# mpieva/network-aware-bwa

Hardware: AMD Instinct MI355X
Metric: aligned reads/s to GRCh38 (100 bp SE), FM-index search (bwa_cal_sa_reg_gap), bit-exact vs CPU (higher is better)
Workload: dtype u32

## Files before the change

include/nabwa.h:

```cpp
#ifndef NABWA_H
#define NABWA_H
#include <stdint.h>
#include <stddef.h>

#ifdef __cplusplus
extern "C" {
#endif

#define NABWA_OK        0
#define NABWA_ENODEV   -1
#define NABWA_EINVAL   -2
#define NABWA_EIO      -3
#define NABWA_ENOMEM   -4
#define NABWA_ECAP     -5
#define NABWA_EHITS    -6

typedef struct {
	int s_mm, s_gapo, s_gape;
	int mode;
	int indel_end_skip, max_del_occ, max_entries;
	float fnr;
	int max_diff, max_gapo, max_gape;
	int max_seed_diff, seed_len;
	int n_threads;
// ... 7 lines not shown
#define NABWA_MODE_NONSTOP  0x10

typedef struct { uint32_t info; uint32_t k, l; int32_t score; } nabwa_aln1_t;

typedef struct nabwa_index nabwa_index_t;

const char *nabwa_last_error(void);
int nabwa_device_count(void);

void nabwa_gap_init_opt(nabwa_gap_opt_t *opt);
int nabwa_cal_maxdiff(int len, double err, double thres);

int nabwa_index_load(const char *prefix, int device, int with_sa, int with_pac, nabwa_index_t **out);

int nabwa_index_from_arrays(int device, int is_device, const uint32_t *bwt0, uint64_t n_words0,
							const uint32_t *bwt1, uint64_t n_words1, const uint32_t *sa0, uint64_t n_sa_words0,
							const uint32_t *sa1, uint64_t n_sa_words1, nabwa_index_t **out);
void nabwa_index_destroy(nabwa_index_t *ix);
uint32_t nabwa_index_seq_len(const nabwa_index_t *ix, int which);
uint64_t nabwa_index_device_bytes(const nabwa_index_t *ix);

int nabwa_cal_sa_reg_gap(nabwa_index_t *ix, const nabwa_gap_opt_t *opt, int n, const int64_t *off,
						 const uint8_t *seq, const uint8_t *rseq, int per_read,
						 int32_t *n_aln, nabwa_aln1_t *aln_out, int64_t aln_cap, int64_t *n_rows,
						 int32_t *max_entries);

typedef struct nabwa_batch nabwa_batch_t;
int nabwa_batch_create(nabwa_index_t *ix, const nabwa_gap_opt_t *opt, int n, const int64_t *off,
					   const uint8_t *seq, const uint8_t *rseq, int per_read, nabwa_batch_t **out);
int nabwa_batch_run(nabwa_batch_t *b);
int nabwa_batch_sync(nabwa_batch_t *b, int *n_second_pass);
float nabwa_batch_last_kernel_ms(nabwa_batch_t *b);
float nabwa_batch_last_width_ms(nabwa_batch_t *b);
float nabwa_batch_last_deep_ms(nabwa_batch_t *b);
int nabwa_batch_count_touches(nabwa_batch_t *b, uint64_t *n_bucket, uint64_t *n_bucket_width);
int nabwa_batch_fetch(nabwa_batch_t *b, int32_t *n_aln, nabwa_aln1_t *aln_out, int64_t aln_cap, int64_t *n_rows,
					  int32_t *max_entries);
int nabwa_batch_width_records(nabwa_batch_t *b, int first, int n, uint32_t *w_out, uint8_t *bid_out, uint8_t *seed_bid_out);
int nabwa_batch_checksum(nabwa_batch_t *b, uint64_t *sum, int64_t *n_rows);
typedef struct {
	int32_t n, min_len, max_len;
	int32_t deep_only;
	int32_t ns1, ns_wide;
	int32_t w_sync;
	int32_t trip_budget, trip_budget_hard;
	int32_t n_sync;
	int32_t hard_budget;
	int32_t cls[3];
	int32_t coop_lanes;
	int32_t lds_rd;
} nabwa_batch_config_t;
int nabwa_batch_config(nabwa_batch_t *b, nabwa_batch_config_t *out);
int nabwa_batch_sure0_stats(nabwa_batch_t *b, uint64_t out[4]);
void nabwa_batch_destroy(nabwa_batch_t *b);

typedef struct { double avg, std, ap_prior; uint32_t low, high, high_bayesian; } nabwa_isize_t;
int nabwa_isize_infer(const uint16_t *hist, double ap_prior, int64_t L, nabwa_isize_t *out);
int nabwa_isize_bin(int kind, int mapq0, int mapq1, uint32_t pos0, int len0, uint32_t pos1, int len1);
typedef struct { uint32_t pos; int32_t strand, mapQ, seQ, len, full_len, n_mm, n_gapo, n_gape, score, extra_flag; } nabwa_pe_end_t;
int nabwa_pairing(nabwa_pe_end_t p[2], int n_hits, uint64_t *hits, const nabwa_aln1_t *rows0, const nabwa_aln1_t *rows1,
				  int max_isize, int s_mm, const nabwa_isize_t *ii);

typedef struct {
	char *name;
	uint8_t *seq, *rseq, *qual;
	uint32_t bits0, bits1;
	int32_t score, clip_len;
	int32_t n_aln; int32_t pad0;
	nabwa_aln1_t *aln;
	int32_t n_multi; int32_t pad1;
	void *multi;
	uint32_t sa, pos;
	uint64_t c1c2seq;
	int32_t n_cigar; int32_t pad2;
	uint16_t *cigar;
	int32_t tid;
	char bc[64];
	uint32_t lenbits;
	char *md;
	int32_t max_entries; int32_t pad3;
} nabwa_bwa_seq_t;

int nabwa_bwa_cal_sa_reg_gap(nabwa_index_t *ix, int n_seqs, nabwa_bwa_seq_t *seqs, const nabwa_gap_opt_t *opt);

int nabwa_encode_read(int full_len, const uint8_t *codes, const uint8_t *qual, int reverse, int trim_qual, int is_comp,
					  uint8_t *seq_out, uint8_t *rseq_out);

int nabwa_sa_lookup(nabwa_index_t *ix, int n, const uint8_t *which, const uint32_t *k, uint32_t *sa_out);

int nabwa_global_align(int device, int n, const int64_t *ref_off, const uint8_t *ref, const int64_t *qry_off,
					   const uint8_t *qry, int gap_open, int gap_ext, int gap_end, const int *matrix25, int band,
					   int32_t *score, int32_t *n_cigar, uint32_t *cigar32, int max_cigar);

void nabwa_dp_scratch_release(int device);

void nabwa_dp_form_counts(uint64_t *out, int n);

int nabwa_extend_align(int device, int n, const int64_t *ref_off, const uint8_t *ref, const int64_t *qry_off,
					   const uint8_t *qry, int gap_open, int gap_ext, const int *matrix25, int band, const int32_t *G0,
					   int32_t *score, int32_t *n_cigar, uint32_t *cigar32, int max_cigar);

int nabwa_local_align(int device, int n, const int64_t *ref_off, const uint8_t *ref, const int64_t *qry_off,
					  const uint8_t *qry, int gap_open, int gap_ext, const int *matrix25, int band, int thres,
					  int32_t *score, int32_t *coords, int32_t *subo, int32_t *n_cigar, uint32_t *cigar32, int max_cigar);

#define NABWA_MAX_CIGAR 64
// ... 176 lines not shown
```

network-aware-bwa_amd/__init__.py:

```python
import ctypes as C
import os
import subprocess

import numpy as np

_HERE = os.path.dirname(os.path.abspath(__file__))
LIB_PATH = os.environ.get("NABWA_LIB", os.path.join(_HERE, "libnabwa.so"))

OK, ENODEV, EINVAL, EIO, ENOMEM, ECAP, EHITS = 0, -1, -2, -3, -4, -5, -6

ALN_DT = np.dtype([("info", "<u4"), ("k", "<u4"), ("l", "<u4"), ("score", "<i4")])


class GapOpt(C.Structure):
    _fields_ = [("s_mm", C.c_int), ("s_gapo", C.c_int), ("s_gape", C.c_int), ("mode", C.c_int),
                ("indel_end_skip", C.c_int), ("max_del_occ", C.c_int), ("max_entries", C.c_int),
                ("fnr", C.c_float), ("max_diff", C.c_int), ("max_gapo", C.c_int), ("max_gape", C.c_int),
                ("max_seed_diff", C.c_int), ("seed_len", C.c_int), ("n_threads", C.c_int),
                ("max_top2", C.c_int), ("trim_qual", C.c_int)]


MAX_CIGAR, MAX_MD, MAX_MULTI = 64, 512, 16


# ... 190 lines not shown
        super().__init__("libnabwa error %d: %s" % (code, msg))
        self.code = code


def build(verbose=False):
    r = subprocess.run(["make", "-C", os.path.join(_HERE, "csrc"), "all"], capture_output=not verbose, text=True)
    if r.returncode != 0:
        raise RuntimeError("building libnabwa.so failed:\n%s\n%s" % (r.stdout, r.stderr))


_lib = None
_P = C.c_void_p


def lib():
    global _lib
    if _lib is not None:
        return _lib
    if not os.path.exists(LIB_PATH):
        raise RuntimeError("libnabwa.so is missing (%s): run __graft_entry__.build() / make -C %s"
                           % (LIB_PATH, os.path.join(_HERE, "csrc")))
    L = C.CDLL(LIB_PATH)
    L.nabwa_last_error.restype = C.c_char_p
    L.nabwa_device_count.restype = C.c_int
    L.nabwa_gap_init_opt.argtypes = [_P]
    L.nabwa_cal_maxdiff.restype = C.c_int
    L.nabwa_cal_maxdiff.argtypes = [C.c_int, C.c_double, C.c_double]
    L.nabwa_index_load.argtypes = [C.c_char_p, C.c_int, C.c_int, C.c_int, _P]
    L.nabwa_index_from_arrays.argtypes = [C.c_int, C.c_int, _P, C.c_uint64, _P, C.c_uint64, _P, C.c_uint64, _P,
                                          C.c_uint64, _P]
    L.nabwa_index_destroy.argtypes = [_P]
    L.nabwa_index_destroy.restype = None
    L.nabwa_index_seq_len.restype = C.c_uint32
    L.nabwa_index_seq_len.argtypes = [_P, C.c_int]
    L.nabwa_index_device_bytes.restype = C.c_uint64
    L.nabwa_index_device_bytes.argtypes = [_P]
    L.nabwa_cal_sa_reg_gap.argtypes = [_P, _P, C.c_int, _P, _P, _P, C.c_int, _P, _P, C.c_int64, _P, _P]
    L.nabwa_batch_create.argtypes = [_P, _P, C.c_int, _P, _P, _P, C.c_int, _P]
    L.nabwa_batch_run.argtypes = [_P]
    L.nabwa_batch_sync.argtypes = [_P, _P]
    L.nabwa_batch_last_kernel_ms.restype = C.c_float
    L.nabwa_batch_last_kernel_ms.argtypes = [_P]
    L.nabwa_batch_last_width_ms.restype = C.c_float
    L.nabwa_batch_last_width_ms.argtypes = [_P]
    L.nabwa_batch_last_deep_ms.restype = C.c_float
    L.nabwa_batch_last_deep_ms.argtypes = [_P]
    L.nabwa_batch_fetch.argtypes = [_P, _P, _P, C.c_int64, _P, _P]
    L.nabwa_batch_checksum.argtypes = [_P, _P, _P]
    L.nabwa_batch_count_touches.argtypes = [_P, _P, _P]
    L.nabwa_batch_config.argtypes = [_P, _P]
    if hasattr(L, "nabwa_batch_sure0_stats"):
        L.nabwa_batch_sure0_stats.restype = C.c_int
        L.nabwa_batch_sure0_stats.argtypes = [_P, _P]
    L.nabwa_dp_form_counts.argtypes = [_P, C.c_int]
    L.nabwa_dp_form_counts.restype = None
    L.nabwa_batch_destroy.argtypes = [_P]
    L.nabwa_batch_destroy.restype = None
    L.nabwa_sa_lookup.argtypes = [_P, C.c_int, _P, _P, _P]
    L.nabwa_occ4.argtypes = [_P, C.c_int, C.c_int, _P, _P]
    L.nabwa_global_align.argtypes = [C.c_int, C.c_int, _P, _P, _P, _P, C.c_int, C.c_int, C.c_int, _P, C.c_int, _P, _P, _P,
                                     C.c_int]
    L.nabwa_extend_align.argtypes = [C.c_int, C.c_int, _P, _P, _P, _P, C.c_int, C.c_int, _P, C.c_int, _P, _P, _P, _P, C.c_int]
    L.nabwa_local_align.argtypes = [C.c_int, C.c_int, _P, _P, _P, _P, C.c_int, C.c_int, _P, C.c_int, C.c_int, _P, _P, _P, _P, _P,
                                    C.c_int]
    L.nabwa_index_attach_reference.argtypes = [_P, C.c_char_p]
    L.nabwa_bwa_cal_sa_reg_gap.argtypes = [_P, C.c_int, _P, _P]
    L.nabwa_isize_infer.argtypes = [_P, C.c_double, C.c_int64, _P]
    L.nabwa_isize_bin.argtypes = [C.c_int, C.c_int, C.c_int, C.c_uint32, C.c_int, C.c_uint32, C.c_int]
    L.nabwa_pairing.argtypes = [_P, C.c_int, _P, _P, _P, C.c_int, C.c_int, _P]
    L.nabwa_encode_read.restype = C.c_int
    L.nabwa_encode_read.argtypes = [C.c_int, _P, _P, C.c_int, C.c_int, C.c_int, _P, _P]
    L.nabwa_se_finish.argtypes = [_P, _P, C.c_int, _P, _P, _P, _P, _P, _P, C.c_int, _P, _P]
    L.nabwa_index_export.argtypes = [_P, C.c_int, C.c_int, C.c_uint64, C.c_uint64, _P]
    L.nabwa_pe_opt_default.argtypes = [_P]
    L.nabwa_pe_opt_default.restype = None
    L.nabwa_pe_posn.argtypes = [_P, _P, C.c_int, _P, _P, _P, _P, _P, _P]
    L.nabwa_pe_finish.argtypes = [_P, _P, _P, _P, C.c_int, _P, _P, _P, _P, _P, _P, _P, _P]
    L.nabwa_index_fa2pac.restype = C.c_int64
    L.nabwa_index_fa2pac.argtypes = [C.c_char_p, C.c_char_p]
    L.nabwa_index_fa2cspac.restype = C.c_int64
    L.nabwa_index_fa2cspac.argtypes = [C.c_char_p, C.c_char_p]
    L.nabwa_index_build.argtypes = [C.c_char_p, C.c_int, C.c_int, C.c_int]
    L.nabwa_index_build_estimate.argtypes = [C.c_uint64, _P]
    L.nabwa_cs2nt.argtypes = [C.c_int, C.c_int, _P, _P, _P, _P]
    L.nabwa_index_attach_nt_reference.argtypes = [_P, C.c_char_p]
    L.nabwa_se_finish_cs.argtypes = [_P, _P, C.c_int, _P, _P, _P, _P, _P, _P, _P, C.c_int, _P, _P, _P, _P, _P, _P]
    L.nabwa_pe_finish_sampe_cs.argtypes = [_P, _P, _P, _P, C.c_int, _P, _P, _P, _P, _P, _P, _P, _P, _P, _P, _P, _P, _P]
    L.nabwa_pairing_typed.argtypes = [_P, C.c_int, _P, _P, _P, C.c_int, C.c_int, _P, C.c_int]
    L.nabwa_bgzf_bound.restype = C.c_int64
    L.nabwa_bgzf_bound.argtypes = [C.c_int64]
    L.nabwa_bgzf_compress.argtypes = [C.c_int, _P, C.c_int64, _P, C.c_int64, _P, _P]
    L.nabwa_bgzf_create.argtypes = [C.c_int, _P]
    L.nabwa_bgzf_handle_compress.argtypes = [_P, _P, C.c_int64, _P, C.c_int64, _P, _P]
    L.nabwa_bgzf_destroy.argtypes = [_P]
    L.nabwa_bgzf_destroy.restype = None
    _lib = L
    return L


def _chk(rc):
    if rc != OK:
        raise NabwaError(rc, lib().nabwa_last_error().decode())


def _ptr(a):
    return a.ctypes.data_as(_P) if a is not None else None
# ... 324 lines not shown
        s = C.c_uint64()
        r = C.c_int64()
        _chk(lib().nabwa_batch_checksum(self._h, C.byref(s), C.byref(r)))
        return s.value, r.value

    def count_touches(self):
        v, w = C.c_uint64(), C.c_uint64()
        _chk(lib().nabwa_batch_count_touches(self._h, C.byref(v), C.byref(w)))
        return v.value, w.value

    def fetch(self):
        n_aln = np.zeros(max(self.n, 1), np.int32)
        maxe = np.zeros(max(self.n, 1), np.int32)
        rows = C.c_int64()
        rc = lib().nabwa_batch_fetch(self._h, _ptr(n_aln), None, 0, C.byref(rows), _ptr(maxe))
        if rc not in (OK, ECAP):
            _chk(rc)
        buf = np.zeros(max(rows.value, 1), ALN_DT)
        if rows.value:
            _chk(lib().nabwa_batch_fetch(self._h, _ptr(n_aln), _ptr(buf), rows.value, C.byref(rows), _ptr(maxe)))
        n_aln = n_aln[:self.n]
        bounds = np.concatenate([[0], np.cumsum(n_aln)])
        return [buf[bounds[i]:bounds[i + 1]] for i in range(self.n)], maxe[:self.n]

    def fetch_flat(self, keep=None):
        if keep is not None and "n_aln" in keep and len(keep["n_aln"]) >= max(self.n, 1):
            n_aln, maxe, buf = keep["n_aln"], keep["maxe"], keep["rows"]
        else:
            n_aln = np.zeros(max(self.n, 1), np.int32)
            maxe = np.zeros(max(self.n, 1), np.int32)
            buf = None
        rows = C.c_int64()
        rc = lib().nabwa_batch_fetch(self._h, _ptr(n_aln), _ptr(buf) if buf is not None else None, len(buf) if buf is not None else 0, C.byref(rows), _ptr(maxe))
        if rc not in (OK, ECAP):
            _chk(rc)
        if rc == ECAP or buf is None:
            buf = np.zeros(max(rows.value + rows.value // 8, 1), ALN_DT)
            if rows.value:
                _chk(lib().nabwa_batch_fetch(self._h, _ptr(n_aln), _ptr(buf), len(buf), C.byref(rows), _ptr(maxe)))
        if keep is not None:
            keep["n_aln"], keep["maxe"], keep["rows"] = n_aln, maxe, buf
        return n_aln[:self.n], buf[:rows.value], maxe[:self.n]

    def config(self):
        c = BatchConfig()
        _chk(lib().nabwa_batch_config(self._h, C.byref(c)))
        return {f: (list(getattr(c, f)) if f == "cls" else getattr(c, f)) for f, _ in BatchConfig._fields_}

    def sure0_stats(self):
        out = (C.c_uint64 * 4)()
        _chk(lib().nabwa_batch_sure0_stats(self._h, out))
        return [int(x) for x in out]

    def close(self):
        if self._h:
            lib().nabwa_batch_destroy(self._h)
            self._h = None
```

network-aware-bwa_amd/csrc/fm_search.hip:

```cpp
#include "nabwa_dev.hpp"
#include "fm_search.hpp"
#include "launchers.hpp"

#define ST_IDLE   0
#define ST_WIDTH  1
#define ST_POP    2
#define ST_EXACT  3
#define ST_EXPAND 4
#define ST_EXIT   5

#define STATE_M 0
#define STATE_I 1
#define STATE_D 2
#define STATE_GROUP 3
#define GRP_EXT 0x100u
#define TXM 0xfffffffeu
#define KEYM 0xffffffffu
#define LVO(t_) ((size_t)((((uint64_t)1 << (2 * (t_))) - 4ull) / 3ull))
#ifndef NABWA_W_WAVES
#define NABWA_W_WAVES 5
#endif
#ifndef NABWA_WORK_CHUNK
#define NABWA_WORK_CHUNK 64u
#endif
// ... 196 lines not shown
				if (kk > ll || cc > 3) { kk = 0; ll = BX(seq_len); ++bid; rekey(wi + 1); }
				else if (was_one) { tmode = true; tp = sav - 1u; twtag = 0xffffffffu; }
			}
			out_pos(wi, false);
			if (wi + 1 == n) out_pos(wi + 1, true);
			++wi;
			if (wi == n) {
				if (phase == 0 && P.rd_cls) P.rd_cls[2 * (size_t)rid + x] = (uint8_t)(bid - 1 > 4 ? 4 : bid - 1);
				if (phase == 0 && len > P.seed_len) {
					phase = 1; wi = 0; n = P.seed_len; sbase = len - P.seed_len; tmode = false;
					if (KT) { wkey = P.rd_key[6 * (size_t)rid + 4 + x]; tok = wkey != 0xffffffffu; }
					tbase = 0;
					kk = 0; ll = BX(seq_len); bid = 0; pw = 0;
				} else { if (x == 0u) P.rd_nN[rid] = (uint8_t)(nN > 255 ? 255 : nN); run = false; }
			}
		}
	}
	if (COUNT) {
		for (int o = 32; o > 0; o >>= 1) touches += __shfl_down(touches, o);
		if (lane == 0 && P.touch_counter) atomicAdd(P.touch_counter + 1, touches);
	}
#undef WREC
#undef BX
}
#define LS_IDLE  0
#define LS_POP   1
#define LS_HAVE  2
#define LS_EXACT 3
#define LS_EXIT  4

template <bool COUNT>
__global__ __launch_bounds__(NABWA_SEARCH_BLOCK, NABWA_MIN_WAVES) void fm_search_kernel(const SearchParams P_)
{
	SearchParams P = P_;
	own(P.n); own(P.s_mm); own(P.s_gapo); own(P.s_gape); own(P.mode); own(P.indel_end_skip); own(P.max_del_occ); own(P.max_entries);
	own(P.max_gape); own(P.max_seed_diff); own(P.seed_len); own(P.max_top2);
	const uint32_t NIL = 0xffffu;
	const uint32_t lane = threadIdx.x & 63u;
	const size_t slot = (size_t)blockIdx.x * NABWA_SEARCH_BLOCK + threadIdx.x;
	uint8_t *const sc = P.scratch + slot * P.lane_stride;
	uint4 *const ent = (uint4*)sc;
	const bool gape_mode = P.mode & 0x01, nonstop = P.mode & 0x10, loggap = P.mode & 0x04;

	int st = LS_IDLE;
	unsigned int w_next = 0, w_end = 0; bool w_sync = false;
	uint32_t item = 0; int len = 0; uint32_t mdmg = 0;
	uint32_t sq_off = 0;
	const int KT = (int)P.bwt[0].kmer_T;
	uint32_t budget = P.trip_budget;
	if (!COUNT && P.n_sync && P.trip_budget_hard && 2u * (uint32_t)__builtin_amdgcn_readfirstlane((int)*P.n_sync) > (uint32_t)P.n) budget = P.trip_budget_hard;
#define RID item
#define REC (P.wdata + (size_t)RID * P.wstride)
#define MD_READ ((int)(mdmg & 0xffu))
#define MG_READ ((int)(mdmg >> 8 & 0x7fu))
	uint32_t k = 0, l = 0;
	int max_diff = 0, best_score = 0, best_cnt = 0, n_aln = 0, max_ent = 0, n_entries = 0;
	uint32_t bump = 0; uint64_t mask_lo = 0; bool seeded = false; int status = 0;
	int e_i = 0, e_a = 0, e_mm = 0, e_go = 0, e_ge = 0, e_state = 0, e_ldp = 0, e_score = 0, m = 0;
	uint4 pe = make_uint4(0, 0, 0, 0); int p_score = -1;
#define p_valid (p_score >= 0)
	int sq_tag = -1;
	int bw_base = -1, bw_a = -1;
	int sw_base = -1, sw_a = -1;
	unsigned long long touches = 0; uint32_t rd_touch = 0, rd_trips = 0;
	uint32_t rk_kf = 0, rk_row2 = 0, rk_row1 = 0, rk_tx = 0, rk_pop = 0, rk_tail = 0, rk_jump = 0, rk_gap = 0;
	unsigned long long st_trips = 0, st_expand = 0, st_exact = 0, st_ent = 0, st_spec = 0, st_query = 0, st_two = 0, st_exit = 0, st_jump = 0, st_txe = 0, st_txt = 0;
	bool ovf = false;
#define s0f mdmg
#define S0_ON  0x80000000u
#define S0_LAND 0x40000000u
#define S0_WAS 0x8000u

	auto head_get = [&](int score) -> uint32_t {
		return (uint32_t)s_head[score * NABWA_SEARCH_BLOCK + threadIdx.x];
	};
	auto head_set = [&](int score, uint32_t v) {
		s_head[score * NABWA_SEARCH_BLOCK + threadIdx.x] = (uint16_t)v;
	};
	auto mask_has = [&](int score) -> bool { return mask_lo >> score & 1ull; };
	auto mask_set = [&](int score) { mask_lo |= 1ull << score; };
	auto mask_clr = [&](int score) { mask_lo &= ~(1ull << score); };
	auto mask_any = [&]() -> bool { return mask_lo != 0ull; };
	auto mask_first = [&]() -> int {
		return mask_lo ? __ffsll((unsigned long long)mask_lo) - 1 : 0x7fffffff;
	};
	auto never_popped = [&](int score) -> bool { return !nonstop && score > best_score + P.s_mm; };
	auto mk_entry = [&](uint32_t nk, uint32_t nl, int ni, int nldp, int nmm, int ngo, int nge, int nstate, int na) -> uint4 {
		const uint32_t z = (uint32_t)ni | (uint32_t)nldp << 16;
		return make_uint4(nk, nl, z, (uint32_t)nmm << 16 | (uint32_t)ngo << 20 | (uint32_t)nge << 24 | (uint32_t)nstate << 29 | (uint32_t)na << 31);
	};
	auto push_mem = [&](int score, uint4 e) {
		if (ovf || never_popped(score)) return;
		if ((uint32_t)score >= P.NS) { ovf = true; return; }
		if (bump >= P.cap) { ovf = true; return; }
		const uint32_t s = bump++;
		const uint32_t prev = mask_has(score) ? head_get(score) : NIL;
		e.w |= prev;
		ent[s] = e;
		head_set(score, s);
		mask_set(score);
	};

	uint4 *const s_pf = (uint4*)(s_head + (size_t)P.NS * NABWA_SEARCH_BLOCK);
	uint2 *const s_key = (uint2*)(s_pf + NABWA_SEARCH_BLOCK);
	uint2 *const s_tw = s_key + NABWA_SEARCH_BLOCK;
	uint32_t *const s_bw = (uint32_t*)(s_tw + NABWA_SEARCH_BLOCK), *const s_sw = s_bw + 4 * NABWA_SEARCH_BLOCK, *const s_sq = s_sw + 4 * NABWA_SEARCH_BLOCK;
	uint32_t *const s_fb = s_sq + 4 * NABWA_SEARCH_BLOCK;
	auto win_byte = [&](const uint32_t *W, uint32_t idx) -> uint32_t {
		return (uint32_t)((const uint8_t*)W)[(threadIdx.x << 4) + idx];
	};
	auto win_load = [&](const void *src, uint32_t *W) {
		__builtin_amdgcn_global_load_lds((const void __attribute__((address_space(1)))*)src,
										 (void __attribute__((address_space(3)))*)(W + ((threadIdx.x & ~63u) << 2)), 16, 0, 0);
	};
#define BW_BYTE(i_) win_byte(s_bw, (uint32_t)(i_))
#define SW_BYTE(i_) win_byte(s_sw, (uint32_t)(i_))
#define SQ_BYTE(i_) win_byte(s_sq, (uint32_t)(i_))
	const bool kf_ok = KT > 0 && (int)P.bwt[0].kmer_LW == KT && (int)P.bwt[1].kmer_LW == KT && (P.text_mode & 4);
	const bool text_ok = (P.text_mode & 2) && P.bwt[0].sa_full && P.bwt[1].sa_full && P.bwt[0].seq_len < 0xfffffff0u;
	uint32_t pf_slot = NIL;
	bool finish = false;
	auto unpack = [&](const uint4 &r) {
		k = r.x; l = r.y; e_i = (int)(r.z & 0xffffu); e_ldp = (int)(r.z >> 16);
		e_mm = (int)(r.w >> 16 & 15u); e_go = (int)(r.w >> 20 & 15u); e_ge = (int)(r.w >> 24 & 31u);
		e_state = (int)(r.w >> 29 & 3u); e_a = (int)(r.w >> 31);
	};
	auto take_entry = [&](const uint4 &r_ent) {
		unpack(r_ent);
		const uint32_t nx = r_ent.w & 0xffffu;
		head_set(e_score, nx);
		if (nx == NIL) mask_clr(e_score);
		--n_entries;
		if (!nonstop && e_score > best_score + P.s_mm) finish = true;
	};

	for (;;) {
		finish = false;
		unsigned long long need = __ballot(st == LS_IDLE);
		const bool any_busy = __ballot(st != LS_IDLE && st != LS_EXIT) != 0ull;
		if ((P.sync_refill || w_sync) && any_busy) need = 0ull;
		if (need) {
			if (w_next == w_end) {
				unsigned int b0 = 0;
				if (lane == 0) b0 = atomicAdd(P.work_counter, (unsigned int)NABWA_WORK_CHUNK);
				w_next = __builtin_amdgcn_readfirstlane(b0); w_end = w_next + NABWA_WORK_CHUNK;
				w_sync = P.n_sync && (w_next >= *P.n_sync || w_next < P.n_sync[-8]);
			}
			const unsigned int rank = (unsigned int)__popcll(need & ((1ull << lane) - 1ull)), avail = w_end - w_next;
			const unsigned int base = w_next;
			w_next += min((unsigned int)__popcll(need), avail);
			if (st == LS_IDLE && rank < avail) {
				const unsigned int idx = base + rank;
				if (idx < (unsigned int)P.n) {
					const uint32_t rid = P.ids ? (uint32_t)P.ids[idx] : idx;
					item = rid;
					const int64_t o = P.poff[rid];
					len = P.rd_len[rid];
					sq_off = (uint32_t)o;
					mdmg = (uint32_t)P.rd_maxdiff[rid] | (uint32_t)P.rd_maxgapo[rid] << 8;
					if (KT) {
						s_key[threadIdx.x] = *(const uint2*)(P.rd_key + 6 * (size_t)rid);
						uint32_t fb = 0xffffu;
						if (len > KT) { const uint8_t *const bb = REC + P.woff_bid + (len - KT - 1); fb = (uint32_t)(bb[0] & 127u) | (uint32_t)(bb[P.WLB] & 127u) << 8; }
						s_fb[threadIdx.x] = fb;
					}
					n_aln = 0; max_ent = 0; status = NABWA_ST_OK; rd_touch = 0; rd_trips = 0; ovf = false;
					rk_kf = rk_row2 = rk_row1 = rk_tx = rk_pop = rk_tail = rk_jump = rk_gap = 0;
					sq_tag = -1; bw_a = -1; sw_a = -1; p_score = -1; pf_slot = NIL;
					if (text_ok) s_tw[threadIdx.x] = make_uint2(0u, 0x7fffffffu);
					if (!COUNT && P.sure0 && P.rd_cls && !nonstop && P.s_gapo > P.s_mm && MD_READ >= 1 && len > 0 && 2 + 4 * len <= P.max_entries) {
						const uint32_t cw = *(const uint16_t*)(P.rd_cls + 2 * (size_t)rid);
						if ((cw & 0xffu) == 0u || (cw >> 8) == 0u) {
							s0f |= P.sure0 > 1 ? S0_ON | S0_LAND | S0_WAS : S0_ON | S0_WAS;
						}
					}
					if (len > 0 && (int)P.rd_nN[rid] <= MD_READ) {
						seeded = len > P.seed_len;
						max_diff = MD_READ;
						best_score = (s0f & S0_ON) ? 0 : (MD_READ + 1) * P.s_mm + (MG_READ + 1) * P.s_gapo + (P.max_gape + 1) * P.s_gape;
						best_cnt = 0;
						bump = 0; mask_lo = 0ull;
						push_mem(0, mk_entry(0u, kf_ok ? KEYM : P.bwt[0].seq_len, len, 0, 0, 0, 0, STATE_M, 0));
						pe = mk_entry(0u, kf_ok ? KEYM : P.bwt[0].seq_len, len, 0, 0, 0, 0, STATE_M, 1); p_score = 0;
						n_entries = 2;
						st = LS_POP;
					} else { P.n_aln[item] = 0; P.max_ent[item] = 0; P.status[item] = NABWA_ST_OK; }
				} else st = LS_EXIT;
			}
		}
		if (__ballot(st != LS_EXIT) == 0ull) break;

		bool want_ent = false; uint32_t ent_slot = 0;
		bool have = st == LS_HAVE;
		if (st == LS_POP) {
			if (n_entries == 0) finish = true;
			else {
				if (max_ent < n_entries) max_ent = n_entries;
				if (n_entries > P.max_entries) finish = true;
				else if (!COUNT && P.trip_budget && rd_trips > budget) { status = NABWA_ST_OVERFLOW; finish = true; }
			}
			if (!finish) {
				const int best_mem = mask_first();
				if (p_valid && p_score <= best_mem) {
					unpack(pe);
					e_score = p_score; p_score = -1;
					--n_entries;
					if (!nonstop && e_score > best_score + P.s_mm) finish = true;
					else have = true;
				} else if (best_mem == 0x7fffffff) {
					finish = true;
				} else {
					if (p_valid) { push_mem(p_score, pe); p_score = -1; }
					if (ovf) { status = NABWA_ST_OVERFLOW; finish = true; }
					else {
						ent_slot = head_get(best_mem); e_score = best_mem;
						if (ent_slot == pf_slot) {
							const uint4 r = s_pf[threadIdx.x];
							take_entry(r);
							pf_slot = NIL;
							if (!finish) have = true;
						} else want_ent = true;
					}
				}
			}
		}
		int kind = 0;
		bool need_win = false, spec = false, forced = false; int win_hi = 0;
		int grp_c = 0, mlev = -1, mpost = 0; uint32_t midx = 0; bool kx = false;
		if (have && !finish && e_state == STATE_GROUP) {
			const uint32_t mk = (uint32_t)e_ldp & 0x1fu, ext = (uint32_t)e_ldp & GRP_EXT, more = (uint32_t)e_ldp >> 9;
			const int j = 31 - __clz((int)mk);
			const uint32_t rest = mk & ~(1u << j);
			if (rest) push_mem(e_score, mk_entry(k, l, e_i, (int)(rest | ext | more << 9), e_mm, e_go, e_ge, STATE_GROUP, e_a));
			else if (more) push_mem(e_score, mk_entry(k + 1u, l, e_i + 1, (int)(3u | (more - 1u) << 9), e_mm, e_go, e_ge, STATE_GROUP, e_a));
			if (ovf) { status = NABWA_ST_OVERFLOW; finish = true; }
			if (ext) ++e_ge; else ++e_go;
			if (l == KEYM) {
				const int dp = len - e_i - 1;
				kind = 6; st = LS_POP; have = false;
				if (j == 0) { mpost = 1; mlev = dp; midx = k; } else { mpost = 2; mlev = dp + 1; midx = k * 4u + (uint32_t)(j - 1); }
			}
			else if (j == 0) { e_state = STATE_I; e_ldp = e_i; }
			else if (l == TXM) { k -= 1u; e_i += 1; e_state = STATE_D; e_ldp = e_i; }
			else { kind = 5; grp_c = j - 1; st = LS_POP; have = false; }
		}
		if (have && !finish) {
			st = LS_POP;
			m = max_diff - (e_mm + e_go); if (gape_mode) m -= e_ge;
			if (m >= 0) {
				const bool kf = l == KEYM;
				const int d = len - e_i;
				if (e_i == 0) { if (kf) { kind = 6; mlev = d; midx = k; } else kind = 3; }
				else {
					const bool tail = m == 0 && (e_state == STATE_M || gape_mode || e_ge == P.max_gape);
					const bool landed = e_state == STATE_M && e_ldp > e_i;
					win_hi = landed ? e_ldp - 1 : e_i - 1;
					const int win_lo = landed ? win_hi : ((tail || e_i < 2) ? e_i - 1 : e_i - 2);
					bool go = true;
					if (bw_a == e_a && win_lo >= bw_base && win_hi < bw_base + 16) {
						if (m < (int)(BW_BYTE(win_hi - bw_base) & 127u)) go = false;
					} else { need_win = true; spec = true; }
					if (go) {
						const bool rdkey_ok = KT && (e_a ? s_key[threadIdx.x].y : s_key[threadIdx.x].x) != 0xffffffffu;
						const bool row_known = l != TXM && !kf && (e_go | e_ge) == 0 && e_state == STATE_M && (e_mm == 0 || (e_mm == 1 && e_ldp == e_i));
						if (tail) {
							kind = 2;
							if (l == TXM) kind = 7;
							else if (kf) { if (rdkey_ok) kind = 4; else { kind = 6; mlev = d; midx = k; } }
							else if (rdkey_ok && row_known && d <= KT) kind = 4;
						}
						else {
							forced = rdkey_ok && d < KT && (kf || row_known) && (int)(s_fb[threadIdx.x] >> (e_a << 3) & 0xffu) == m;
							if (forced) kind = 4;
							else if (kf && d >= KT) { kind = 6; mlev = d; midx = k; }
							else {
								kind = 1; --e_i; kx = kf;
								if ((s0f & S0_ON) && n_entries + 4 * len > P.max_entries) s0f &= ~S0_ON;
							}
						}
					}
				}
			}
		} else if (st == LS_EXACT) kind = l == TXM ? 7 : 2;
		auto rows_arrived = [&](uint32_t nk, uint32_t nl) {
			k = nk; l = nl;
			if (mpost == 1) { e_state = STATE_I; e_ldp = e_i; }
			else if (mpost == 2) { e_i += 1; e_state = STATE_D; e_ldp = e_i; }
			st = LS_HAVE;
		};
		if (kind == 6 && mlev == 0) { rows_arrived(0u, e_a ? P.bwt[0].seq_len : P.bwt[1].seq_len); kind = 0; }

		const int qb = 1 - e_a;
		const bool tx = l == TXM && (kind == 1 || kind == 3 || kind == 7);
		const int spos = (kind == 2 || kind == 7) ? e_i - 1 : e_i;
		const int stag = (e_a << 20) | (spos >> 4);
		const bool need_seq = (kind == 1 || kind == 2 || kind == 7) && stag != sq_tag;
		bool query = (kind == 1 && !tx && !kx) || kind == 2 || kind == 5;
		uint2 tw = make_uint2(0u, 0u); bool need_tw = false;
		if (tx && kind != 3 && k > 0u) {
			const uint32_t tag = ((k - 1u) >> 4) | (uint32_t)qb << 31;
			tw = s_tw[threadIdx.x];
			need_tw = tw.y != tag;
			tw.y = tag;
		}
		const bool to_text = kind == 1 && !tx && !kx && text_ok && k == l;
		if (kind == 2 && !need_seq && SQ_BYTE((uint32_t)spos & 15u) > 3u) query = false;
		const int ii = e_i - (len - P.seed_len);
		const bool use_seed = kind == 1 && e_i > 0 && seeded && ii > 0;
		const bool need_seed = use_seed && !(sw_a == e_a && ii - 1 >= sw_base && ii < sw_base + 16);

		uint4 r_ent = make_uint4(0, 0, 0, 0);
		if (need_win) {
			int base = (win_hi | 7) - 15; if (base < 0) base = 0;
			win_load(REC + P.woff_bid + e_a * P.WLB + base, s_bw); bw_base = base; bw_a = e_a;
		}
		if (need_seq) {
			win_load((e_a ? P.rseq : P.seq) + sq_off + (spos & ~15), s_sq); sq_tag = stag;
		}
		if (need_seed) {
			int base = (ii | 7) - 15; if (base < 0) base = 0;
			win_load(REC + P.woff_sbid + e_a * P.SLB + base, s_sw); sw_base = base; sw_a = e_a;
		}
		uint32_t r_x = 0u;
		if (need_tw) r_x = (qb ? P.bwt[1].text : P.bwt[0].text)[(k - 1u) >> 4];
		else if (tx && kind == 3) r_x = (qb ? P.bwt[1].isa : P.bwt[0].isa)[k];
		else if (to_text) r_x = (qb ? P.bwt[1].sa_full : P.bwt[0].sa_full)[k];
		uint2 r_km = make_uint2(1u, 0u);
		uint4 a0, a1, a2, a3, b0, b1, b2, b3;
// ... 276 lines not shown
								ek = gk; el = gl; ei = len - KT; s0f += 1u << 23;
							}
						}
						if (dead) ++n_entries;
						else emit(sc0 + (is_mm ? P.s_mm : 0), ek, el, ei, is_mm ? e_i : 0, e_mm + (is_mm ? 1 : 0), e_go, e_ge, STATE_M, 1);
						if (!is_mm) match_child = true;
					}
				}
			} else if (c < 4) {
				const uint32_t nk = L2Q(c) + CK(c) + 1u, nl = L2Q(c) + CL(c);
				if (nk <= nl) { emit(sc0, nk, nl, e_i, 0, e_mm, e_go, e_ge, STATE_M, 1); match_child = true; }
			}
			if (to_text && match_child) { pe.x = r_x - 1u; pe.y = TXM; }
			if (ovf) { status = NABWA_ST_OVERFLOW; finish = true; }
		}
#undef L2Q
#undef CK
#undef CL

		if (finish) {
			const bool net = (s0f & S0_ON) && status == NABWA_ST_OK && n_aln == 0;
			if (net) status = NABWA_ST_OVERFLOW;
			if (P.s0_stats && (s0f & S0_WAS)) atomicAdd(P.s0_stats, 1ull);
			if (P.s0_stats && (s0f >> 16 & 0x3fffu)) {
				atomicAdd(P.s0_stats + 1, (unsigned long long)(s0f >> 16 & 0x7fu)); atomicAdd(P.s0_stats + 2, (unsigned long long)(s0f >> 23 & 0x7fu));
			}
			if (P.s0_stats && net) atomicAdd(P.s0_stats + 3, 1ull);
			P.n_aln[item] = n_aln; P.max_ent[item] = (!COUNT && status == NABWA_ST_OVERFLOW) ? (int)rd_trips : max_ent; P.status[item] = (uint8_t)status;
			if (COUNT && status == NABWA_ST_OK) touches += rd_touch;
			if (COUNT && P.touch_counter && rd_trips > 8000u) {
				atomicAdd(P.touch_counter + 16, 1ull); atomicAdd(P.touch_counter + 17, (unsigned long long)rd_trips); atomicAdd(P.touch_counter + 18, (unsigned long long)rk_kf);
				atomicAdd(P.touch_counter + 19, (unsigned long long)rk_row2); atomicAdd(P.touch_counter + 20, (unsigned long long)rk_row1); atomicAdd(P.touch_counter + 21, (unsigned long long)rk_tx);
				atomicAdd(P.touch_counter + 22, (unsigned long long)rk_pop); atomicAdd(P.touch_counter + 23, (unsigned long long)rk_tail); atomicAdd(P.touch_counter + 24, (unsigned long long)rk_jump); atomicAdd(P.touch_counter + 25, (unsigned long long)rk_gap);
			}
			if (COUNT && P.touch_counter) { atomicMax(P.touch_counter + 13, (unsigned long long)rd_trips); if (rd_trips > 2000u) atomicAdd(P.touch_counter + 14, 1ull); if (rd_trips > 500u) atomicAdd(P.touch_counter + 15, 1ull); }
			st = LS_IDLE;
		}
	}
	if (COUNT) {
		for (int o = 32; o > 0; o >>= 1) touches += __shfl_down(touches, o);
		if (lane == 0 && P.touch_counter) {
			atomicAdd(P.touch_counter, touches);
			atomicAdd(P.touch_counter + 2, st_trips); atomicAdd(P.touch_counter + 3, st_expand); atomicAdd(P.touch_counter + 4, st_exact);
			atomicAdd(P.touch_counter + 5, st_ent); atomicAdd(P.touch_counter + 6, st_spec); atomicAdd(P.touch_counter + 7, st_query);
			atomicAdd(P.touch_counter + 8, st_two); atomicAdd(P.touch_counter + 9, st_exit); atomicAdd(P.touch_counter + 10, st_jump); atomicAdd(P.touch_counter + 11, st_txe); atomicAdd(P.touch_counter + 12, st_txt);
		}
	}
}

#undef p_valid
#undef S0_ON
#undef S0_LAND
#undef S0_WAS
#undef s0f
#undef BW_BYTE
#undef SW_BYTE
#undef SQ_BYTE
#undef RID
#undef REC
#undef MD_READ
#undef MG_READ
extern "C" void nabwa_launch_fm_width(const SearchParams *P, int n_blocks, hipStream_t s)
{
	if (P->touch_counter) hipLaunchKernelGGL((fm_width_kernel<true>), dim3(n_blocks), dim3(NABWA_SEARCH_BLOCK), 0, s, *P);
	else hipLaunchKernelGGL((fm_width_kernel<false>), dim3(n_blocks), dim3(NABWA_SEARCH_BLOCK), 0, s, *P);
}

extern "C" int nabwa_width_occupancy(void)
{
	int nb = 0;
	return hipOccupancyMaxActiveBlocksPerMultiprocessor(&nb, fm_width_kernel<false>, NABWA_SEARCH_BLOCK, 0) == hipSuccess ? nb : 0;
}

extern "C" void nabwa_launch_fm_search(const SearchParams *P, int n_blocks, hipStream_t s)
{
	const size_t lds = (size_t)P->NS * NABWA_SEARCH_BLOCK * 2 + NABWA_SEARCH_BLOCK * 84;
	if (P->touch_counter) hipLaunchKernelGGL((fm_search_kernel<true>), dim3(n_blocks), dim3(NABWA_SEARCH_BLOCK), lds, s, *P);
	else hipLaunchKernelGGL((fm_search_kernel<false>), dim3(n_blocks), dim3(NABWA_SEARCH_BLOCK), lds, s, *P);
}

extern "C" int nabwa_search_occupancy(int ns)
{
	int nb = 0;
	hipError_t e = hipOccupancyMaxActiveBlocksPerMultiprocessor(&nb, fm_search_kernel<false>, NABWA_SEARCH_BLOCK,
																(size_t)ns * NABWA_SEARCH_BLOCK * 2 + NABWA_SEARCH_BLOCK * 84);
	return e == hipSuccess ? nb : 0;
}

__global__ __launch_bounds__(256) void pad_reads_kernel(int n, const uint8_t *__restrict__ seq, const uint8_t *__restrict__ rseq,
													const int64_t *__restrict__ off, const int64_t *__restrict__ poff,
													uint8_t *__restrict__ pseq, uint8_t *__restrict__ prseq, int32_t *__restrict__ rd_len,
													uint32_t *__restrict__ rd_key, int T, int seed_len, uint32_t *__restrict__ rd_pack, int pack_stride,
													const uint8_t *__restrict__ md_tab, const uint8_t *__restrict__ mg_tab,
													uint8_t *__restrict__ rd_md, uint8_t *__restrict__ rd_mg)
{
	const int t = threadIdx.x & 15;
	const int i = blockIdx.x * 16 + (threadIdx.x >> 4);
	if (i >= n) return;
	const int64_t o = off[i], p = poff[i];
	const int L = (int)(off[i + 1] - o), NC = (int)(poff[i + 1] - p) >> 4;
	if (t == 0) { rd_len[i] = L; rd_md[i] = md_tab[L]; rd_mg[i] = mg_tab[L]; }
	const int PW = pack_stride / 2;
	uint32_t *const pk = rd_pack ? rd_pack + (size_t)i * pack_stride : 0;
	const int n_turns = pk && PW - 1 > NC ? PW - 1 : NC;
	uint32_t anyN[2] = { 0u, 0u };
	for (int c = t; c < n_turns; c += 16) {
// ... 270 lines not shown
```

network-aware-bwa_amd/csrc/nabwa_batch.hip:

```cpp
#include <hip/hip_runtime.h>
#include <hipcub/hipcub.hpp>
#include <stdio.h>
#include <stdlib.h>
#include <string.h>
#include <memory>
#include <vector>
#include "../../include/nabwa.h"
#include "nabwa_batch.hpp"
#include "host_util.hpp"

static void layout(SearchParams &P, uint32_t cap, int max_len, int seed_len, uint32_t NS)
{
	P.WL = align_up((uint32_t)max_len + 1, 16);
	P.WLB = P.WL + 16;
	P.SLB = align_up((uint32_t)(max_len > seed_len ? seed_len : 0) + 1, 16) + 16;
	P.woff_bid = 2 * P.WL * 4;
	P.woff_sbid = P.woff_bid + 2 * P.WLB;
	P.wstride = align_up(P.woff_sbid + 2 * P.SLB, 64);
	P.cap = cap; P.NS = NS;
	P.lane_stride = align_up((size_t)cap * 16, 64);
}

extern "C" void nabwa_batch_destroy(nabwa_batch_t *b)
{
// ... 94 lines not shown
	const double tu0 = now_s();
	HIP_CHECK(staged_upload(ix, jobs, 3));
	if (timing) fprintf(stderr, "[nabwa] upload of %.2f GB: %.3f s (%.3f s into batch_create)\n", 2e-9 * (double)off[n], now_s() - tu0, tu0 - tc0);
	HIP_CHECK(plen.get(ix, (size_t)(n + 1) * 8));
	nabwa_launch_padded_len(n, raw_off, plen, b->stream);
	HIP_CHECK(hipcub::DeviceScan::ExclusiveSum(nullptr, tmp_bytes, plen.p, b->d_poff.p, n + 1, b->stream));
	HIP_CHECK(d_tmp.get(ix, tmp_bytes ? tmp_bytes : 16));
	HIP_CHECK(hipcub::DeviceScan::ExclusiveSum(d_tmp.p, tmp_bytes, plen.p, b->d_poff.p, n + 1, b->stream));
	HIP_CHECK(d_tab.get(ix, 2 * (size_t)(max_len + 1)));
	HIP_CHECK(hipMemcpyAsync(d_tab, s.md_tab.data(), max_len + 1, hipMemcpyHostToDevice, b->stream));
	HIP_CHECK(hipMemcpyAsync(d_tab + max_len + 1, s.mg_tab.data(), max_len + 1, hipMemcpyHostToDevice, b->stream));
	nabwa_launch_pad_reads(n, raw_s, raw_r, raw_off, b->d_poff, b->d_seq, b->d_rseq, b->d_len, b->d_key,
						   ix->bwt[0].kmer_T == ix->bwt[1].kmer_T ? (int)ix->bwt[0].kmer_T : 0, b->opt.seed_len, b->d_pack, b->pack_stride,
						   d_tab, d_tab + max_len + 1, b->d_md, b->d_mg, b->stream);
	HIP_CHECK(hipStreamSynchronize(b->stream));
	if (timing) fprintf(stderr, "[nabwa] re-layout kernel done %.3f s into batch_create\n", now_s() - tc0);
	HIP_CHECK(raw_s.release()); HIP_CHECK(raw_r.release()); HIP_CHECK(raw_off.release());
	HIP_CHECK(plen.release()); HIP_CHECK(d_tmp.release()); HIP_CHECK(d_tab.release());
	return NABWA_OK;
}

static int working_buffers(nabwa_batch *b, const BatchShape &s)
{
	nabwa_index *ix = b->ix;
	const nabwa_gap_opt_t *opt = &b->opt;
	const int n = b->n, max_len = s.max_len;
	SearchParams &P = b->P;
	memset(&P, 0, sizeof(P));
	P.bwt[0] = ix->bwt[0]; P.bwt[1] = ix->bwt[1];
	{
		uint32_t tab[NABWA_IXTAB_WORDS];
		nabwa_ixtab_fill(tab, ix->bwt);
		HIP_CHECK(b->d_ixtab.get(ix, sizeof tab));
		HIP_CHECK(hipMemcpy(b->d_ixtab, tab, sizeof tab, hipMemcpyHostToDevice));
		P.ixtab = b->d_ixtab;
	}
	P.seq = b->d_seq; P.rseq = b->d_rseq; P.poff = b->d_poff; P.rd_len = b->d_len; P.rd_maxdiff = b->d_md; P.rd_maxgapo = b->d_mg; P.rd_key = b->d_key; P.rd_pack = b->d_pack; P.pack_stride = b->pack_stride;
	P.text_mode = env_int("NABWA_TEXT_KERNELS", 7);
	if (ix->bwt[0].kmer_T != ix->bwt[1].kmer_T) P.bwt[0].kmer_T = P.bwt[1].kmer_T = 0;
	P.ids = 0; P.n = n;
	P.s_mm = opt->s_mm; P.s_gapo = opt->s_gapo; P.s_gape = opt->s_gape; P.mode = opt->mode;
	P.indel_end_skip = opt->indel_end_skip; P.max_del_occ = opt->max_del_occ; P.max_entries = opt->max_entries;
	P.max_gape = opt->max_gape; P.max_seed_diff = opt->max_seed_diff; P.seed_len = opt->seed_len; P.max_top2 = opt->max_top2;
	int cap1 = env_int("NABWA_CAP1", 4096);
	if (cap1 < 16) cap1 = 16;
	if (cap1 > 65534) cap1 = 65534;
	layout(P, (uint32_t)cap1, max_len, opt->seed_len, s.deep_only ? 1u : s.NS1);
	P.aln_cap = env_int("NABWA_ALNCAP1", 16);
	P.sync_refill = env_int("NABWA_SYNC_REFILL", 0);
	P.trip_budget = (uint32_t)env_int("NABWA_TRIP_BUDGET", max_len > opt->seed_len ? 2000 : 300);
	P.trip_budget_hard = (uint32_t)env_int("NABWA_TRIP_BUDGET_HARD", max_len > opt->seed_len ? 200 : (int)P.trip_budget);
	if (getenv("NABWA_TRIP_BUDGET") && !getenv("NABWA_TRIP_BUDGET_HARD")) P.trip_budget_hard = P.trip_budget;
	b->class_sort = env_int("NABWA_CLASS_SORT", 1);
	P.sure0 = env_int("NABWA_SURE0", 2);
	if (P.sure0 < 0) P.sure0 = 0;
	if (P.sure0 > 2) P.sure0 = 2;
	if (env_int("NABWA_SURE0_STATS", 0)) {
		HIP_CHECK(b->d_s0stats.get(ix, 32));
		HIP_CHECK(hipMemset(b->d_s0stats, 0, 32));
		P.s0_stats = b->d_s0stats;
	}
	{
		P.w_sync = (n > 0 && s.min_len == max_len) ? env_int("NABWA_W_SYNC", 1) : 0;
	}
	if (P.aln_cap < 1) P.aln_cap = 1;

	hipDeviceProp_t prop;
	HIP_CHECK(hipGetDeviceProperties(&prop, ix->device));
	int occ = nabwa_search_occupancy(s.deep_only ? 1 : (int)s.NS1);
	if (occ < 1) occ = 1;
	const int occ_env = env_int("NABWA_BLOCKS_PER_CU", 0);
	if (occ_env > 0) occ = occ_env;
	long blocks = (long)prop.multiProcessorCount * occ;
	const long need = ((long)n + NABWA_SEARCH_BLOCK - 1) / NABWA_SEARCH_BLOCK;
	if (blocks > need) blocks = need;
	if (blocks < 1) blocks = 1;
	b->n_blocks = (int)blocks;
	if (getenv("NABWA_TIMING")) fprintf(stderr, "[nabwa] search kernel: %u score levels, %d blocks per CU (LDS %zu B per block), %ld blocks\n", s.NS1, occ,
										(size_t)s.NS1 * NABWA_SEARCH_BLOCK * 2 + NABWA_SEARCH_BLOCK * 80, blocks);
	HIP_CHECK(b->d_scratch.get(ix, (size_t)blocks * NABWA_SEARCH_BLOCK * P.lane_stride));
	int occw = nabwa_width_occupancy(); if (occw < 1) occw = 1;
	long blocks_w = (long)prop.multiProcessorCount * occw;
	if (blocks_w > 2 * need) blocks_w = 2 * need;
	if (blocks_w < 1) blocks_w = 1;
	b->n_blocks_w = (int)blocks_w;
	HIP_CHECK(b->d_wdata.get(ix, (size_t)(n ? n : 1) * P.wstride));
	HIP_CHECK(b->d_nN.get(ix, n ? n : 1));
	P.wdata = b->d_wdata; P.rd_nN = b->d_nN;
	const size_t n1 = n ? n : 1;
	HIP_CHECK(b->d_naln.get(ix, n1 * 4)); HIP_CHECK(b->d_maxent.get(ix, n1 * 4)); HIP_CHECK(b->d_wide_idx.get(ix, n1 * 4));
	HIP_CHECK(b->d_status.get(ix, n1)); HIP_CHECK(b->d_aln.get(ix, n1 * (size_t)P.aln_cap * 16));
	HIP_CHECK(b->d_counter.get(ix, 16)); HIP_CHECK(b->d_novf.get(ix, 4)); HIP_CHECK(b->d_ovf_ids.get(ix, n1 * 4));
	HIP_CHECK(b->d_sum.get(ix, 256));
	P.scratch = b->d_scratch; P.n_aln = b->d_naln; P.max_ent = b->d_maxent; P.status = b->d_status; P.aln = b->d_aln;
	P.work_counter = b->d_counter;
	return NABWA_OK;
}

extern "C" int nabwa_batch_create(nabwa_index_t *ix, const nabwa_gap_opt_t *opt, int n, const int64_t *off,
								  const uint8_t *seq, const uint8_t *rseq, int per_read, nabwa_batch_t **out)
{
	if (!ix || !opt || !off || !out || n < 0 || (n && (!seq || !rseq))) return nabwa_fail(NABWA_EINVAL, "null argument");
	HIP_CHECK(hipSetDevice(ix->device));
	const bool timing = getenv("NABWA_TIMING") != 0;
	const double tc0 = now_s();
	BatchShape s;
	if (int r = derive_options(opt, n, off, per_read, s)) return r;

	const double tc1 = now_s();
	std::unique_ptr<nabwa_batch, void (*)(nabwa_batch*)> b(new nabwa_batch(), nabwa_batch_destroy);
	b->ix = ix; b->opt = *opt; b->n = n; b->deep_only = s.deep_only ? 1 : 0;
	b->max_len = s.max_len; b->min_len = n ? s.min_len : 0; b->NS1 = s.NS1; b->NS_wide = s.NS; b->deep_coop = -1;
// ... 178 lines not shown
}

extern "C" int nabwa_batch_checksum(nabwa_batch_t *b, uint64_t *sum, int64_t *n_rows)
{
	if (!b) return nabwa_fail(NABWA_EINVAL, "null batch");
	HIP_CHECK(hipSetDevice(b->ix->device));
	unsigned long long h[2] = { 0, 0 };
	HIP_CHECK(hipMemsetAsync(b->d_sum, 0, 16, b->stream));
	nabwa_launch_checksum(b->n, b->d_naln, b->d_aln, b->P.aln_cap, b->d_status, b->d_wide_idx, b->d_aln2, b->aln_cap2, b->d_grown_tab,
						  b->d_sum, b->d_sum + 1, b->stream);
	HIP_CHECK(hipMemcpyAsync(h, b->d_sum, 16, hipMemcpyDeviceToHost, b->stream));
	HIP_CHECK(hipStreamSynchronize(b->stream));
	if (sum) *sum = h[0];
	if (n_rows) *n_rows = (int64_t)h[1];
	return NABWA_OK;
}

extern "C" int nabwa_batch_config(nabwa_batch_t *b, nabwa_batch_config_t *out)
{
	if (!b || !out) return nabwa_fail(NABWA_EINVAL, "null argument");
	memset(out, 0, sizeof(*out));
	out->n = b->n; out->min_len = b->min_len; out->max_len = b->max_len;
	out->deep_only = b->deep_only; out->ns1 = (int32_t)b->NS1; out->ns_wide = (int32_t)b->NS_wide;
	out->w_sync = b->P.w_sync; out->trip_budget = (int32_t)b->P.trip_budget; out->trip_budget_hard = (int32_t)b->P.trip_budget_hard;
	out->n_sync = out->hard_budget = -1;
	for (int q = 0; q < 3; ++q) out->cls[q] = -1;
	if (b->ran && b->class_sort) {
		HIP_CHECK(hipSetDevice(b->ix->device));
		unsigned int c[12];
		HIP_CHECK(hipMemcpyAsync(c, b->d_ncls, 48, hipMemcpyDeviceToHost, b->stream));
		HIP_CHECK(hipStreamSynchronize(b->stream));
		for (int q = 0; q < 3; ++q) out->cls[q] = (int32_t)c[q];
		out->n_sync = (int32_t)c[10];
		if (!b->deep_only) out->hard_budget = b->P.trip_budget_hard && 2u * c[10] > (uint32_t)b->n ? 1 : 0;
	}
	out->coop_lanes = b->deep_coop;
	out->lds_rd = b->deep_cfg ? (int32_t)b->deep_lds_rd : -1;
	return NABWA_OK;
}

extern "C" int nabwa_batch_sure0_stats(nabwa_batch_t *b, uint64_t out[4])
{
	if (!b || !out) return nabwa_fail(NABWA_EINVAL, "null argument");
	for (int q = 0; q < 4; ++q) out[q] = 0;
	if (!b->d_s0stats) return NABWA_OK;
	HIP_CHECK(hipSetDevice(b->ix->device));
	unsigned long long v[4];
	HIP_CHECK(hipMemcpyAsync(v, b->d_s0stats, 32, hipMemcpyDeviceToHost, b->stream));
	HIP_CHECK(hipStreamSynchronize(b->stream));
	for (int q = 0; q < 4; ++q) out[q] = v[q];
	return NABWA_OK;
}

extern "C" int nabwa_batch_fetch(nabwa_batch_t *b, int32_t *n_aln, nabwa_aln1_t *aln_out, int64_t aln_cap, int64_t *n_rows,
								 int32_t *max_entries)
{
	if (!b || !n_aln) return nabwa_fail(NABWA_EINVAL, "null argument");
	HIP_CHECK(hipSetDevice(b->ix->device));
	if (n_rows) *n_rows = 0;
	if (b->n == 0) return NABWA_OK;
	PoolBuf<uint32_t> d_off; PoolBuf<void> d_tmp; size_t tmp_bytes = 0; PoolBuf<uint4> d_rows;
	StreamDrain drain{ b->stream };
	HIP_CHECK(d_off.get(b->ix, (size_t)(b->n + 1) * 4));
	HIP_CHECK(hipcub::DeviceScan::ExclusiveSum(nullptr, tmp_bytes, (const uint32_t*)b->d_naln.p, d_off.p, b->n, b->stream));
	HIP_CHECK(d_tmp.get(b->ix, tmp_bytes ? tmp_bytes : 16));
	HIP_CHECK(hipcub::DeviceScan::ExclusiveSum(d_tmp.p, tmp_bytes, (const uint32_t*)b->d_naln.p, d_off.p, b->n, b->stream));
	uint32_t last_off = 0; int32_t last_n = 0;
	HIP_CHECK(hipMemcpyAsync(&last_off, d_off + (b->n - 1), 4, hipMemcpyDeviceToHost, b->stream));
	HIP_CHECK(hipMemcpyAsync(&last_n, b->d_naln + (b->n - 1), 4, hipMemcpyDeviceToHost, b->stream));
	HIP_CHECK(hipMemcpyAsync(n_aln, b->d_naln, (size_t)b->n * 4, hipMemcpyDeviceToHost, b->stream));
	if (max_entries) HIP_CHECK(hipMemcpyAsync(max_entries, b->d_maxent, (size_t)b->n * 4, hipMemcpyDeviceToHost, b->stream));
	HIP_CHECK(hipStreamSynchronize(b->stream));
	const int64_t total = (int64_t)last_off + last_n;
	if (n_rows) *n_rows = total;
	int rc = NABWA_OK;
	if (total > aln_cap || (total && !aln_out)) rc = nabwa_fail(NABWA_ECAP, "aln_cap too small");
	else if (total) {
		HIP_CHECK(d_rows.get(b->ix, (size_t)total * 16));
		nabwa_launch_gather(b->n, b->d_naln, d_off, b->d_aln, b->P.aln_cap, b->d_status, b->d_wide_idx, b->d_aln2, b->aln_cap2, b->d_grown_tab,
							d_rows, b->stream);
		HIP_CHECK(hipMemcpyAsync(aln_out, d_rows, (size_t)total * 16, hipMemcpyDeviceToHost, b->stream));
		HIP_CHECK(hipStreamSynchronize(b->stream));
		HIP_CHECK(d_rows.release());
	}
	HIP_CHECK(d_off.release()); HIP_CHECK(d_tmp.release());
	return rc;
}
```

Measured before the change: 98.33 million.

## Add sure0 level 3 shortcut collapsing exact-match prefix walk in search

Adds a new sure0 mode (now the default) that, when a read's class word shows zero mismatches for a strand, skips the per-base exact-match stepping. It jumps the position counter to zero in one step and analytically accounts for the gap entries that would have been pushed. The goal is to remove many FM-index iterations on clean reads while keeping entry and max_ent bookkeeping bit-exact. It also narrows the MG_READ field mask and extends the stats buffer and API for new counters. If the analytic entry accounting differs from the real walk, bit-exactness is at risk.

```diff
diff --git a/include/nabwa.h b/include/nabwa.h
--- a/include/nabwa.h
+++ b/include/nabwa.h
@@ -83,6 +83,7 @@
 } nabwa_batch_config_t;
 int nabwa_batch_config(nabwa_batch_t *b, nabwa_batch_config_t *out);
 int nabwa_batch_sure0_stats(nabwa_batch_t *b, uint64_t out[4]);
+int nabwa_batch_sure0_stats_ex(nabwa_batch_t *b, uint64_t out[8]);
 void nabwa_batch_destroy(nabwa_batch_t *b);
 
 typedef struct { double avg, std, ap_prior; uint32_t low, high, high_bayesian; } nabwa_isize_t;
diff --git a/network-aware-bwa_amd/__init__.py b/network-aware-bwa_amd/__init__.py
--- a/network-aware-bwa_amd/__init__.py
+++ b/network-aware-bwa_amd/__init__.py
@@ -266,6 +266,9 @@
     if hasattr(L, "nabwa_batch_sure0_stats"):
         L.nabwa_batch_sure0_stats.restype = C.c_int
         L.nabwa_batch_sure0_stats.argtypes = [_P, _P]
+    if hasattr(L, "nabwa_batch_sure0_stats_ex"):
+        L.nabwa_batch_sure0_stats_ex.restype = C.c_int
+        L.nabwa_batch_sure0_stats_ex.argtypes = [_P, _P]
     L.nabwa_dp_form_counts.argtypes = [_P, C.c_int]
     L.nabwa_dp_form_counts.restype = None
     L.nabwa_batch_destroy.argtypes = [_P]
@@ -696,6 +699,11 @@
         _chk(lib().nabwa_batch_sure0_stats(self._h, out))
         return [int(x) for x in out]
 
+    def sure0_stats_ex(self):
+        out = (C.c_uint64 * 8)()
+        _chk(lib().nabwa_batch_sure0_stats_ex(self._h, out))
+        return [int(x) for x in out]
+
     def close(self):
         if self._h:
             lib().nabwa_batch_destroy(self._h)
diff --git a/network-aware-bwa_amd/csrc/fm_search.hip b/network-aware-bwa_amd/csrc/fm_search.hip
--- a/network-aware-bwa_amd/csrc/fm_search.hip
+++ b/network-aware-bwa_amd/csrc/fm_search.hip
@@ -272,7 +272,7 @@
 #define RID item
 #define REC (P.wdata + (size_t)RID * P.wstride)
 #define MD_READ ((int)(mdmg & 0xffu))
-#define MG_READ ((int)(mdmg >> 8 & 0x7fu))
+#define MG_READ ((int)(mdmg >> 8 & 0xfu))
 	uint32_t k = 0, l = 0;
 	int max_diff = 0, best_score = 0, best_cnt = 0, n_aln = 0, max_ent = 0, n_entries = 0;
 	uint32_t bump = 0; uint64_t mask_lo = 0; bool seeded = false; int status = 0;
@@ -290,6 +290,7 @@
 #define S0_ON  0x80000000u
 #define S0_LAND 0x40000000u
 #define S0_WAS 0x8000u
+#define S0_PRV 0x1000u
 
 	auto head_get = [&](int score) -> uint32_t {
 		return (uint32_t)s_head[score * NABWA_SEARCH_BLOCK + threadIdx.x];
@@ -392,6 +393,7 @@
 						const uint32_t cw = *(const uint16_t*)(P.rd_cls + 2 * (size_t)rid);
 						if ((cw & 0xffu) == 0u || (cw >> 8) == 0u) {
 							s0f |= P.sure0 > 1 ? S0_ON | S0_LAND | S0_WAS : S0_ON | S0_WAS;
+							if (P.sure0 > 2) s0f |= ((cw & 0xffu) == 0u ? S0_PRV : 0u) | ((cw >> 8) == 0u ? S0_PRV << 1 : 0u);
 						}
 					}
 					if (len > 0 && (int)P.rd_nN[rid] <= MD_READ) {
@@ -493,7 +495,22 @@
 							forced = rdkey_ok && d < KT && (kf || row_known) && (int)(s_fb[threadIdx.x] >> (e_a << 3) & 0xffu) == m;
 							if (forced) kind = 4;
 							else if (kf && d >= KT) { kind = 6; mlev = d; midx = k; }
+							else if (l == TXM && (s0f & S0_ON) && (s0f & S0_PRV << e_a) && e_state == STATE_M && (e_mm | e_go | e_ge) == 0
+									 && n_entries + 4 * len <= P.max_entries && k >= (uint32_t)e_i) {
+								const int ies = P.indel_end_skip + (loggap ? 1 : 0);
+								int hi = e_i - 1;
+								if (hi > len - ies) hi = len - ies;
+								if (seeded && P.max_seed_diff < 1 && hi > len - P.seed_len) hi = len - P.seed_len;
+								const int gl = (MG_READ > 0 && hi >= ies) ? hi - ies + 1 : 0;
+								if (P.s0_stats) { atomicAdd(P.s0_stats + 4, 1ull); atomicAdd(P.s0_stats + 5, (unsigned long long)e_i); }
+								n_entries += 2 * gl;
+								if (max_ent < n_entries + 1) max_ent = n_entries + 1;
+								k -= (uint32_t)e_i; e_i = 0; e_ldp = 0;
+								kind = 3; need_win = false; spec = false;
+							}
 							else {
+								if (P.s0_stats && l == TXM && (s0f & S0_ON) && (s0f & S0_PRV << e_a) && e_state == STATE_M && (e_mm | e_go | e_ge) == 0
+									&& n_entries + 4 * len <= P.max_entries) atomicAdd(P.s0_stats + 6, 1ull);
 								kind = 1; --e_i; kx = kf;
 								if ((s0f & S0_ON) && n_entries + 4 * len > P.max_entries) s0f &= ~S0_ON;
 							}
@@ -876,6 +893,7 @@
 #undef S0_ON
 #undef S0_LAND
 #undef S0_WAS
+#undef S0_PRV
 #undef s0f
 #undef BW_BYTE
 #undef SW_BYTE
diff --git a/network-aware-bwa_amd/csrc/nabwa_batch.hip b/network-aware-bwa_amd/csrc/nabwa_batch.hip
--- a/network-aware-bwa_amd/csrc/nabwa_batch.hip
+++ b/network-aware-bwa_amd/csrc/nabwa_batch.hip
@@ -170,12 +170,12 @@
 	P.trip_budget_hard = (uint32_t)env_int("NABWA_TRIP_BUDGET_HARD", max_len > opt->seed_len ? 200 : (int)P.trip_budget);
 	if (getenv("NABWA_TRIP_BUDGET") && !getenv("NABWA_TRIP_BUDGET_HARD")) P.trip_budget_hard = P.trip_budget;
 	b->class_sort = env_int("NABWA_CLASS_SORT", 1);
-	P.sure0 = env_int("NABWA_SURE0", 2);
+	P.sure0 = env_int("NABWA_SURE0", 3);
 	if (P.sure0 < 0) P.sure0 = 0;
-	if (P.sure0 > 2) P.sure0 = 2;
+	if (P.sure0 > 3) P.sure0 = 3;
 	if (env_int("NABWA_SURE0_STATS", 0)) {
-		HIP_CHECK(b->d_s0stats.get(ix, 32));
-		HIP_CHECK(hipMemset(b->d_s0stats, 0, 32));
+		HIP_CHECK(b->d_s0stats.get(ix, 64));
+		HIP_CHECK(hipMemset(b->d_s0stats, 0, 64));
 		P.s0_stats = b->d_s0stats;
 	}
 	{
@@ -460,6 +460,19 @@
 	return NABWA_OK;
 }
 
+extern "C" int nabwa_batch_sure0_stats_ex(nabwa_batch_t *b, uint64_t out[8])
+{
+	if (!b || !out) return nabwa_fail(NABWA_EINVAL, "null argument");
+	for (int q = 0; q < 8; ++q) out[q] = 0;
+	if (!b->d_s0stats) return NABWA_OK;
+	HIP_CHECK(hipSetDevice(b->ix->device));
+	unsigned long long v[8];
+	HIP_CHECK(hipMemcpyAsync(v, b->d_s0stats, 64, hipMemcpyDeviceToHost, b->stream));
+	HIP_CHECK(hipStreamSynchronize(b->stream));
+	for (int q = 0; q < 8; ++q) out[q] = v[q];
+	return NABWA_OK;
+}
+
 extern "C" int nabwa_batch_fetch(nabwa_batch_t *b, int32_t *n_aln, nabwa_aln1_t *aln_out, int64_t aln_cap, int64_t *n_rows,
 								 int32_t *max_entries)
 {
```

After: 103.3 million (median of 6 runs). 5.0% higher.
